# christhetree/mod_extraction

Measured on AMD Instinct MI355X. Metric: 44.1 kHz audio-seconds/sec (train step), interwoven ph/fl/ch, higher is better.
Workload: dtype f32

## Files before the change

mod_extraction_amd/csrc/phaser.hip:

```cpp
#include "phaser_common.h"

#define PH_BLOCK 256
#define PH_WPB 4

__global__ __launch_bounds__(64 * PH_WPB) void phaser_kernel(const float *__restrict__ x, long long x_stride,
                                                    const float *__restrict__ rate,
                                                    const float *__restrict__ depth,
                                                    const float *__restrict__ centre,
                                                    const float *__restrict__ feedback,
                                                    const float *__restrict__ mix,
                                                    const int *__restrict__ lead_arr,
                                                    const int *__restrict__ rows, int n_items, int N,
                                                    double sr, float *__restrict__ y, long long y_stride,
                                                    float *__restrict__ dry_out)
{
    const int lane = threadIdx.x & 63;
    const int item = blockIdx.x * PH_WPB + (threadIdx.x >> 6);
    if (item >= n_items) return;
    const int b = rows ? rows[item] : item;
    const int lead = lead_arr ? lead_arr[b] : 0;
    const int total = lead + N;
    const float *xb = x + (size_t)b * x_stride;
    float *yb = y + (size_t)b * y_stride;
    float *db = dry_out ? dry_out + (size_t)b * y_stride : nullptr;

    const PsClip k = ps_clip(sr, rate[b], depth[b], centre[b], feedback[b], mix[b]);

    float phase = 0.0f;
    float z[7] = {0.f, 0.f, 0.f, 0.f, 0.f, 0.f, 0.f};

    for (int n0 = 0; n0 < total; n0 += PH_BLOCK) {
        float xr[PH_BLOCK / 64], yr[PH_BLOCK / 64];
#pragma unroll
        for (int j = 0; j < PH_BLOCK / 64; ++j) {
            const int n = n0 + j * 64 + lane;
            xr[j] = n < total ? xb[n] : 0.0f;
            yr[j] = 0.0f;
        }
        float my_phase = 0.0f;
        for (int u = 0; u < PH_BLOCK / 4; ++u) {
            if (lane == u) my_phase = phase;
            phase = ps_step(phase, k.inc);
        }
        float pre_unused;
        const float Greg = ps_cutoff(k, ps_osc(my_phase), pre_unused);
        const int cnt = min(PH_BLOCK, total - n0);
#pragma unroll
        for (int j = 0; j < PH_BLOCK / 64; ++j) {
            const int lim = min(64, cnt - j * 64);
            for (int li = 0; li < lim; ++li) {
                const float in = __int_as_float(__builtin_amdgcn_readlane(__float_as_int(xr[j]), li));
                const float G = __int_as_float(__builtin_amdgcn_readlane(__float_as_int(Greg), (j * 64 + li) >> 2));
                const float out = ps_sample(G, k.fb, in, z);
                float m = __fadd_rn(__fmul_rn(out, k.wet_g), __fmul_rn(in, k.dry_g));
                m = m < -1.0f ? -1.0f : (m > 1.0f ? 1.0f : m);
                yr[j] = lane == li ? m : yr[j];
            }
        }
#pragma unroll
        for (int j = 0; j < PH_BLOCK / 64; ++j) {
            const int n = n0 + j * 64 + lane;
            if (n >= lead && n < total) {
                yb[n - lead] = yr[j];
                if (db) db[n - lead] = xr[j];
            }
        }
    }
}


__device__ float ps_phase_after(int g, float inc)
{
    const float two_pi = PS_TWO_PI;
    float p = 0.0f;
    int rem = g;
    while (rem > 0) {
        const float p1 = ps_step(p, inc);
        p = p1;
        if (--rem == 0) break;
        const float p2 = ps_step(p1, inc);
        p = p2;
        if (--rem == 0) break;
        const float p3 = ps_step(p2, inc);
        p = p3;
        if (--rem == 0) break;
        const float d1 = __fsub_rn(p2, p1), d2 = __fsub_rn(p3, p2);
        const int e1 = (__float_as_int(p1) >> 23) & 0xff, e2 = (__float_as_int(p2) >> 23) & 0xff, e3 = (__float_as_int(p3) >> 23) & 0xff;
        if (d1 == d2 && d2 > 0.0f && e1 == e2 && e2 == e3 && e3 > 0 && e3 < 0xfe) {
            const double edge = (double)__int_as_float((e3 + 1) << 23);
            const double lim = edge < (double)two_pi ? edge : (double)two_pi;
            long long j = (long long)floor((lim - (double)p3) / (double)d2) - 1;
            if (j > rem) j = rem;
            if (j > 0) {
                p = (float)((double)p3 + (double)j * (double)d2);
                rem -= (int)j;
            }
        }
    }
    return p;
}

template <bool STASH>
__global__ __launch_bounds__(PS_P) void phaser_scan_kernel(const float *__restrict__ x, long long x_stride,
                                                           const float *__restrict__ rate,
                                                           const float *__restrict__ depth,
                                                           const float *__restrict__ centre,
                                                           const float *__restrict__ feedback,
                                                           const float *__restrict__ mix,
                                                           const int *__restrict__ lead_arr,
                                                           const int *__restrict__ rows, int n_items, int N, double sr,
                                                           float *__restrict__ y, long long y_stride,
                                                           float *__restrict__ dry_out, float *__restrict__ gws,
                                                           long long gws_stride, int probe,
                                                           const float *__restrict__ mod, long long mod_stride, int n_mod,
                                                           float *__restrict__ stash, long long stash_stride, int sg,
                                                           int x_width)
{
    extern __shared__ __attribute__((aligned(16))) float ps_lds[];
    float *mv = ps_lds, *zs = ps_lds + PS_P * PS_MV;
    const int p = threadIdx.x, lane = p & 63;
    const int item = blockIdx.x;
    const int b = rows ? rows[item] : item;
    const int lead = lead_arr ? lead_arr[b] : 0;
    const int total = lead + N;
    const float *xb = x + (size_t)b * x_stride;
    float *yb = y + (size_t)b * y_stride;
    float *db = dry_out ? dry_out + (size_t)b * y_stride : nullptr;
    float *gw = gws + (size_t)item * gws_stride;
    PsStash<float> st = {nullptr, sg};
    const float *mb = nullptr;
    if constexpr (STASH) {
        if (total > x_width || ((total + 3) >> 2) > sg) return;
        st.row = stash + (size_t)b * stash_stride;
        gw = st.G();
        if (mod) mb = mod + (size_t)b * mod_stride;
    }
    const bool ext = STASH && mb != nullptr;

    const PsClip k = ps_clip(sr, ext ? 0.0f : rate[b], depth[b], centre[b], feedback[b], mix[b]);

    const int n_groups = (total + 3) >> 2;
    const int gpc = (n_groups + PS_P - 1) / PS_P;
    const int g0 = p * gpc, g1 = min(g0 + gpc, n_groups);

    const bool use_ws = STASH || (gws != nullptr && (long long)n_groups <= gws_stride);

    float S[8][7];
#pragma unroll
    for (int r = 0; r < 8; ++r)
#pragma unroll
        for (int c = 0; c < 7; ++c) S[r][c] = r == c ? 1.0f : 0.0f;
    float phase = ext ? 0.0f : ps_phase_after(min(g0, n_groups), k.inc);
    for (int g = g0; g < g1; ++g) {
        float xv[4];
#pragma unroll
        for (int j = 0; j < 4; ++j) {
            const int n = 4 * g + j;
            xv[j] = probe ? 0.25f : (n < total ? xb[n] : 0.0f);
        }
        float pre;
        const float osc = ext ? __fsub_rn(1.0f, __fmul_rn(2.0f, g < n_mod ? mb[g] : 0.5f)) : ps_osc(phase);
        const float G = ps_cutoff(k, osc, pre);
        if constexpr (STASH) {
            st.pre()[g] = pre;
            st.osc()[g] = osc;
        }
        phase = ps_step(phase, k.inc);
        if (use_ws) gw[g] = G;
#pragma unroll
        for (int j = 0; j < 4; ++j) {
#pragma unroll
            for (int r = 0; r < 8; ++r) (void)ps_sample(G, k.fb, r == 7 ? xv[j] : 0.0f, S[r]);
        }
    }
    {
        float *m = mv + p * PS_MV;
#pragma unroll
        for (int c = 0; c < 7; ++c)
#pragma unroll
            for (int r = 0; r < 7; ++r) m[c * 7 + r] = S[c][r];
#pragma unroll
        for (int r = 0; r < 7; ++r) m[49 + r] = S[7][r];
        if constexpr (STASH) m[PS_MV - 1] = 0.0f;
    }
    __syncthreads();

    if (p < 64) {
        const int r = lane < 7 ? lane : 0;
        float z[7], mine = 0.0f;
#pragma unroll
        for (int c = 0; c < 7; ++c) z[c] = 0.0f;
        for (int q = 0; q < PS_P; ++q) {
            if (lane < 7) zs[q * 8 + lane] = mine;
            const float *m = mv + q * PS_MV;
            float acc = m[49 + r];
#pragma unroll
            for (int c = 0; c < 7; ++c) acc = __builtin_fmaf(m[c * 7 + r], z[c], acc);
            mine = acc;
#pragma unroll
            for (int c = 0; c < 7; ++c) z[c] = __int_as_float(__builtin_amdgcn_readlane(__float_as_int(acc), c));
        }
    }
    __syncthreads();
    if constexpr (STASH) {
        for (int i = p; i < PS_P * PS_MV; i += PS_P) st.maps()[i] = mv[i];
        for (int g = n_groups + p; g < sg; g += PS_P) {
            st.G()[g] = 0.0f;
            st.pre()[g] = 0.0f;
            st.osc()[g] = 0.0f;
            st.pass()[g] = 0;
        }
        const float4 zero4 = make_float4(0.0f, 0.0f, 0.0f, 0.0f);
        const int spc = (gpc + PS_SUB - 1) / PS_SUB;
        for (int sub = (max(g1 - g0, 0) + PS_SUB - 1) / PS_SUB; sub < spc; ++sub) {
            float4 *ck = st.ckpt(p, gpc, sub);
            ck[0] = zero4;
            ck[1] = zero4;
        }
        float4 *ck_all = st.ckpt(0, gpc, 0);
        const long long ck_used = 2ll * PS_P * spc, ck_row = 2ll * PS_P * ps_ckpts_per_chunk(sg);
        for (long long i = ck_used + p; i < ck_row; i += PS_P) ck_all[i] = zero4;
    }

    {
        float z[7];
#pragma unroll
        for (int c = 0; c < 7; ++c) z[c] = zs[p * 8 + c];
        float phase_c = use_ws ? 0.0f : ps_phase_after(min(g0, n_groups), k.inc);
        for (int g = g0; g < g1; ++g) {
            float G;
            if (use_ws) G = gw[g];
            else {
                float pre_unused;
                G = ps_cutoff(k, ps_osc(phase_c), pre_unused);
                phase_c = ps_step(phase_c, k.inc);
            }
            float xv[4];
#pragma unroll
            for (int j = 0; j < 4; ++j) {
                const int n = 4 * g + j;
                xv[j] = probe ? 0.25f : (n < total ? xb[n] : 0.0f);
            }
            int passed = 0;
            if constexpr (STASH) {
                if (((g - g0) & (PS_SUB - 1)) == 0) {
                    float4 *ck = st.ckpt(p, gpc, (g - g0) / PS_SUB);
                    ck[0] = make_float4(z[0], z[1], z[2], z[3]);
                    ck[1] = make_float4(z[4], z[5], z[6], 0.0f);
                }
            }
#pragma unroll
            for (int j = 0; j < 4; ++j) {
                const int n = 4 * g + j;
                const float in = xv[j];
                const float out = ps_sample(G, k.fb, in, z);
                float m = __fadd_rn(__fmul_rn(out, k.wet_g), __fmul_rn(in, k.dry_g));
                if constexpr (STASH) passed |= (m >= -1.0f && m <= 1.0f) ? 1 << j : 0;
                m = m < -1.0f ? -1.0f : (m > 1.0f ? 1.0f : m);
                if (n >= lead && n < total && (!probe || g + 1 == g1)) {
                    yb[n - lead] = m;
                    if (db) db[n - lead] = in;
                }
            }
            if constexpr (STASH) st.pass()[g] = passed;
        }
    }
}

static int phaser_fwd_launch(const float *x, int64_t x_stride, const float *rate, const float *depth,
                            const float *centre, const float *feedback, const float *mix, const int32_t *lead,
                            const int32_t *rows, int64_t n_rows, int64_t B, int64_t N, double sr, int32_t exact_order,
                            float *y, int64_t y_stride, float *dry_out, float *workspace, int64_t workspace_stride,
                            void *stream, int probe)
{
    if (!x || !rate || !depth || !centre || !feedback || !mix || !y || B <= 0 || N <= 0 || sr <= 0.0) return MX_ERR_ARG;
    if (workspace && workspace_stride <= 0) return MX_ERR_ARG;
    if (N >= (1ll << 30)) return MX_ERR_UNSUPPORTED;
    const int64_t items = rows ? n_rows : B;
    if (items <= 0) return MX_OK;
    if (exact_order) {
        const dim3 grid((unsigned)((items + PH_WPB - 1) / PH_WPB)), block(64 * PH_WPB);
        hipLaunchKernelGGL(phaser_kernel, grid, block, 0, (hipStream_t)stream, x, (long long)x_stride, rate, depth, centre,
                           feedback, mix, lead, rows, (int)items, (int)N, sr, y, (long long)y_stride, dry_out);
    } else {
        const size_t lds = PS_LDS_FLOATS * sizeof(float);
        static MxLdsLatch latch = {};
        if (mx_set_dyn_lds(latch, (const void *)phaser_scan_kernel<false>, lds) != MX_OK) return MX_ERR_LAUNCH;
        hipLaunchKernelGGL(phaser_scan_kernel<false>, dim3((unsigned)items), dim3(PS_P), lds, (hipStream_t)stream, x, (long long)x_stride,
                           rate, depth, centre, feedback, mix, lead, rows, (int)items, (int)N, sr, y, (long long)y_stride,
                           dry_out, workspace, (long long)workspace_stride, probe, (const float *)nullptr, 0ll, 0,
                           (float *)nullptr, 0ll, 0, 0);
    }
    return mx_launch_status();
}

MX_EXPORT int mx_phaser_fwd(const float *x, int64_t x_stride, const float *rate, const float *depth,
                            const float *centre, const float *feedback, const float *mix, const int32_t *lead,
                            const int32_t *rows, int64_t n_rows, int64_t B, int64_t N, double sr, int32_t exact_order,
                            float *y, int64_t y_stride, float *dry_out, float *workspace, int64_t workspace_stride,
                            void *stream)
{
    return phaser_fwd_launch(x, x_stride, rate, depth, centre, feedback, mix, lead, rows, n_rows, B, N, sr, exact_order, y, y_stride, dry_out, workspace, workspace_stride, stream, 0);
}

MX_EXPORT int mx_phaser_fwd_stash(const float *x, int64_t x_stride, int64_t x_width, const float *mod, int64_t n_mod,
                                  const float *rate, const float *depth, const float *centre, const float *feedback,
                                  const float *mix, const int32_t *lead, const int32_t *rows, int64_t n_rows, int64_t B,
                                  int64_t N, double sr, float *y, int64_t y_stride, float *dry_out, float *stash,
                                  int64_t stash_groups, int64_t stash_stride, void *stream)
{
    if (!x || !(mod || rate) || !depth || !centre || !feedback || !mix || !y || !stash || B <= 0 || N <= 0 || sr <= 0.0)
        return MX_ERR_ARG;
    if (x_width < N || x_stride < x_width || y_stride < N || (mod && n_mod < (x_width + 3) / 4)) return MX_ERR_ARG;
    if (x_width >= (1ll << 30)) return MX_ERR_UNSUPPORTED;
    if (stash_groups < (x_width + 3) / 4 || (stash_groups & 3) || stash_stride < ps_stash_floats(stash_groups)) return MX_ERR_ARG;
    if ((stash_stride & 3) || ((uintptr_t)stash & 15)) return MX_ERR_ARG;
    const int64_t items = rows ? n_rows : B;
    if (items <= 0) return MX_OK;
    const size_t lds = PS_LDS_FLOATS * sizeof(float);
    static MxLdsLatch latch = {};
    if (mx_set_dyn_lds(latch, (const void *)phaser_scan_kernel<true>, lds) != MX_OK) return MX_ERR_LAUNCH;
    hipLaunchKernelGGL(phaser_scan_kernel<true>, dim3((unsigned)items), dim3(PS_P), lds, (hipStream_t)stream, x, (long long)x_stride,
                       rate, depth, centre, feedback, mix, lead, rows, (int)items, (int)N, sr, y, (long long)y_stride, dry_out,
                       (float *)nullptr, 0ll, 0, mod, (long long)n_mod, (int)n_mod, stash, (long long)stash_stride,
                       (int)stash_groups, (int)x_width);
    return mx_launch_status();
}

MX_EXPORT int mx_phaser_fwd_probe(const float *x, int64_t x_stride, const float *rate, const float *depth,
                            const float *centre, const float *feedback, const float *mix, const int32_t *lead,
                            const int32_t *rows, int64_t n_rows, int64_t B, int64_t N, double sr, int32_t exact_order,
                            float *y, int64_t y_stride, float *dry_out, float *workspace, int64_t workspace_stride,
                            void *stream)
{
    return phaser_fwd_launch(x, x_stride, rate, depth, centre, feedback, mix, lead, rows, n_rows, B, N, sr, exact_order, y, y_stride, dry_out, workspace, workspace_stride, stream, 1);
}

__global__ __launch_bounds__(PS_P) void phaser_cascade_probe_kernel(int steps, float G, float fb, float *__restrict__ out)
{
    float s[8][6], last[8];
#pragma unroll
    for (int r = 0; r < 8; ++r) {
        last[r] = 0.0f;
#pragma unroll
        for (int k = 0; k < 6; ++k) s[r][k] = (r == k) ? 1.0f : 0.001f * (float)(threadIdx.x & 7);
    }
    float in = 0.25f + 1e-3f * (float)(threadIdx.x & 15);
    for (int t = 0; t < steps; ++t) {
#pragma unroll
        for (int r = 0; r < 8; ++r) {
            float o = __fsub_rn(r == 7 ? in : 0.0f, last[r]);
#pragma unroll
            for (int k = 0; k < 6; ++k) (void)ps_stage(G, s[r][k], o);
            last[r] = __fmul_rn(o, fb);
        }
        in = -in;
    }
    float acc = 0.0f;
#pragma unroll
    for (int r = 0; r < 8; ++r) acc += last[r] + s[r][5];
    if (acc == 123.456f) out[threadIdx.x] = acc;
    if (threadIdx.x == 0) out[0] = acc;
}

MX_EXPORT int mx_phaser_cascade_probe(int64_t steps, float *out, void *stream)
{
    if (!out || steps <= 0 || steps >= (1ll << 30)) return MX_ERR_ARG;
    hipLaunchKernelGGL(phaser_cascade_probe_kernel, dim3(1), dim3(PS_P), 0, (hipStream_t)stream, (int)steps, 0.37f, 0.45f, out);
    return mx_launch_status();
}
```

mod_extraction_amd/csrc/phaser_common.h:

```cpp
#pragma once
#include "common.h"

#define PS_WAVES 8
#define PS_P (64 * PS_WAVES)
#define PS_MV 57
#define PS_LDS_FLOATS (PS_P * PS_MV + (PS_P + 1) * 8)
#define PS_SUB 2

__host__ __device__ inline long long ps_ckpts_per_chunk(long long n_groups)
{
    const long long gpc = (n_groups + PS_P - 1) / PS_P;
    return (gpc + PS_SUB - 1) / PS_SUB;
}
__host__ __device__ inline long long ps_stash_floats(long long sg)
{
    return 4 * sg + (long long)PS_P * PS_MV + (long long)PS_P * 8 * ps_ckpts_per_chunk(sg);
}

__device__ __forceinline__ int *ps_as_int(float *p) { return reinterpret_cast<int *>(p); }
__device__ __forceinline__ const int *ps_as_int(const float *p) { return reinterpret_cast<const int *>(p); }
__device__ __forceinline__ float4 *ps_as_float4(float *p) { return reinterpret_cast<float4 *>(p); }
__device__ __forceinline__ const float4 *ps_as_float4(const float *p) { return reinterpret_cast<const float4 *>(p); }
template <typename F>
struct PsStash {
    F *row;
    int sg;
    __device__ __forceinline__ F *G() const { return row; }
    __device__ __forceinline__ F *pre() const { return row + sg; }
    __device__ __forceinline__ F *osc() const { return row + 2 * (size_t)sg; }
    __device__ __forceinline__ auto pass() const { return ps_as_int(row) + 3 * (size_t)sg; }
    __device__ __forceinline__ F *maps() const { return row + 4 * (size_t)sg; }
    __device__ __forceinline__ auto ckpt(int p, int gpc, int sub) const
    {
        return ps_as_float4(maps() + PS_P * PS_MV) + 2 * ((size_t)p * ((gpc + PS_SUB - 1) / PS_SUB) + sub);
    }
};

constexpr float PS_TWO_PI = 6.283185307179586476925286766559f;
constexpr double PS_PI = 3.14159265358979323846;

struct PsClip {
    double sr;
    float log_min, span, inc, norm_centre, osc_vol, fb, wet_g, dry_g;
};
__device__ __forceinline__ PsClip ps_clip(double sr, float rate, float depth, float centre, float feedback, float mix)
{
    PsClip k;
    const float fmax_hz = (float)fmin(20000.0, 0.49 * sr);
    k.sr = sr;
    k.log_min = (float)log10(20.0);
    k.span = __fsub_rn((float)log10((double)fmax_hz), k.log_min);
    k.inc = __fmul_rn(__fdiv_rn(PS_TWO_PI, (float)(sr / 4.0)), rate);
    k.norm_centre = __fdiv_rn(__fsub_rn((float)log10((double)centre), k.log_min), k.span);
    k.osc_vol = __fmul_rn(depth, 0.5f);
    k.fb = feedback;
    k.wet_g = mix;
    k.dry_g = __fsub_rn(1.0f, mix);
    return k;
}

__device__ __forceinline__ float ps_step(float p, float inc)
{
    p = __fadd_rn(p, inc);
    while (p >= PS_TWO_PI) p = __fsub_rn(p, PS_TWO_PI);
    return p;
}
__device__ __forceinline__ float ps_osc(float phase) { return (float)sin((double)__fsub_rn(phase, (float)PS_PI)); }
__device__ __forceinline__ float ps_cutoff(const PsClip &k, float osc, float &pre)
{
    pre = __fadd_rn(__fmul_rn(osc, k.osc_vol), k.norm_centre);
    const float lfo = pre < 0.0f ? 0.0f : (pre > 1.0f ? 1.0f : pre);
    const float fc = (float)pow(10.0, (double)__fadd_rn(__fmul_rn(lfo, k.span), k.log_min));
    const float g = (float)tan(PS_PI * (double)fc / k.sr);
    return __fdiv_rn(g, __fadd_rn(1.0f, g));
}

__device__ __forceinline__ float ps_stage(float G, float &s, float &out)
{
    const float d = __fsub_rn(out, s);
    const float v = __fmul_rn(G, d);
    const float yk = __fadd_rn(v, s);
    s = __fadd_rn(v, yk);
    out = __fsub_rn(__fmul_rn(2.0f, yk), out);
    return d;
}
__device__ __forceinline__ float ps_sample(float G, float fb, float in, float (&z)[7], float *d = nullptr)
{
    float out = __fsub_rn(in, z[6]);
#pragma unroll
    for (int k = 0; k < 6; ++k) {
        const float dk = ps_stage(G, z[k], out);
        if (d) d[k] = dk;
    }
    z[6] = __fmul_rn(out, fb);
    return out;
}
```

Baseline: 7651.

## Precompute phaser cutoff table in a separate parallel kernel before scan

Adds a phaser_cutoff_kernel that fills the per-group cutoff coefficient table across a 2D grid, with each thread handling a short run of groups from a recomputed phase. The non-stash scan kernel then reads G from this table (prefetching the next value) instead of evaluating the double-precision sin/pow/tan chain inline. This moves the expensive transcendental work off the serial scan into a wide parallel pass. The cost is an extra launch and a global write/read of the table. In probe mode a fixed constant G stands in for the table.

New measurement: 7649 (median of 2 runs). No clear change (-0.0%).

```diff
diff --git a/mod_extraction_amd/csrc/phaser.hip b/mod_extraction_amd/csrc/phaser.hip
--- a/mod_extraction_amd/csrc/phaser.hip
+++ b/mod_extraction_amd/csrc/phaser.hip
@@ -42,8 +42,7 @@
             if (lane == u) my_phase = phase;
             phase = ps_step(phase, k.inc);
         }
-        float pre_unused;
-        const float Greg = ps_cutoff(k, ps_osc(my_phase), pre_unused);
+        const float Greg = ps_cutoff_at(k, my_phase);
         const int cnt = min(PH_BLOCK, total - n0);
 #pragma unroll
         for (int j = 0; j < PH_BLOCK / 64; ++j) {
@@ -100,6 +99,37 @@
     return p;
 }
 
+#define PC_BLOCK 256
+#define PC_RUN 8
+#define PS_PROBE_G 0.37f
+__global__ __launch_bounds__(PC_BLOCK) void phaser_cutoff_kernel(const float *__restrict__ rate,
+                                                                 const float *__restrict__ depth,
+                                                                 const float *__restrict__ centre,
+                                                                 const float *__restrict__ feedback,
+                                                                 const float *__restrict__ mix,
+                                                                 const int *__restrict__ lead_arr,
+                                                                 const int *__restrict__ rows, int N, double sr,
+                                                                 float *__restrict__ gws, long long gws_stride)
+{
+    const int item = blockIdx.x;
+    const int b = rows ? rows[item] : item;
+    const int lead = lead_arr ? lead_arr[b] : 0;
+    const int total = lead + N;
+    const int n_groups = (total + 3) >> 2;
+    if ((long long)n_groups > gws_stride) return;
+    float *gw = gws + (size_t)item * gws_stride;
+    const PsClip k = ps_clip(sr, rate[b], depth[b], centre[b], feedback[b], mix[b]);
+    const long long span = (long long)gridDim.y * (PC_BLOCK * PC_RUN);
+    for (long long first = ((long long)blockIdx.y * PC_BLOCK + threadIdx.x) * PC_RUN; first < n_groups; first += span) {
+        const int g0 = (int)first, g1 = min(g0 + PC_RUN, n_groups);
+        float phase = ps_phase_after(g0, k.inc);
+        for (int g = g0; g < g1; ++g) {
+            gw[g] = ps_cutoff_at(k, phase);
+            phase = ps_step(phase, k.inc);
+        }
+    }
+}
+
 template <bool STASH>
 __global__ __launch_bounds__(PS_P) void phaser_scan_kernel(const float *__restrict__ x, long long x_stride,
                                                            const float *__restrict__ rate,
@@ -144,13 +174,15 @@
     const int g0 = p * gpc, g1 = min(g0 + gpc, n_groups);
 
     const bool use_ws = STASH || (gws != nullptr && (long long)n_groups <= gws_stride);
+    const bool table = !STASH && use_ws;
 
     float S[8][7];
 #pragma unroll
     for (int r = 0; r < 8; ++r)
 #pragma unroll
         for (int c = 0; c < 7; ++c) S[r][c] = r == c ? 1.0f : 0.0f;
-    float phase = ext ? 0.0f : ps_phase_after(min(g0, n_groups), k.inc);
+    float phase = (ext || table) ? 0.0f : ps_phase_after(min(g0, n_groups), k.inc);
+    float G_next = (table && !probe && g0 < g1) ? gw[g0] : PS_PROBE_G;
     for (int g = g0; g < g1; ++g) {
         float xv[4];
 #pragma unroll
@@ -158,15 +190,21 @@
             const int n = 4 * g + j;
             xv[j] = probe ? 0.25f : (n < total ? xb[n] : 0.0f);
         }
-        float pre;
-        const float osc = ext ? __fsub_rn(1.0f, __fmul_rn(2.0f, g < n_mod ? mb[g] : 0.5f)) : ps_osc(phase);
-        const float G = ps_cutoff(k, osc, pre);
-        if constexpr (STASH) {
-            st.pre()[g] = pre;
-            st.osc()[g] = osc;
-        }
-        phase = ps_step(phase, k.inc);
-        if (use_ws) gw[g] = G;
+        float G;
+        if (table) {
+            G = G_next;
+            if (!probe && g + 1 < g1) G_next = gw[g + 1];
+        } else {
+            float pre;
+            const float osc = ext ? __fsub_rn(1.0f, __fmul_rn(2.0f, g < n_mod ? mb[g] : 0.5f)) : ps_osc(phase);
+            G = ps_cutoff(k, osc, pre);
+            if constexpr (STASH) {
+                st.pre()[g] = pre;
+                st.osc()[g] = osc;
+                gw[g] = G;
+            }
+            phase = ps_step(phase, k.inc);
+        }
 #pragma unroll
         for (int j = 0; j < 4; ++j) {
 #pragma unroll
@@ -229,10 +267,9 @@
         float phase_c = use_ws ? 0.0f : ps_phase_after(min(g0, n_groups), k.inc);
         for (int g = g0; g < g1; ++g) {
             float G;
-            if (use_ws) G = gw[g];
+            if (use_ws) G = (table && probe) ? PS_PROBE_G : gw[g];
             else {
-                float pre_unused;
-                G = ps_cutoff(k, ps_osc(phase_c), pre_unused);
+                G = ps_cutoff_at(k, phase_c);
                 phase_c = ps_step(phase_c, k.inc);
             }
             float xv[4];
@@ -286,6 +323,12 @@
         const size_t lds = PS_LDS_FLOATS * sizeof(float);
         static MxLdsLatch latch = {};
         if (mx_set_dyn_lds(latch, (const void *)phaser_scan_kernel<false>, lds) != MX_OK) return MX_ERR_LAUNCH;
+        if (workspace && !probe) {
+            const int64_t per_block = PC_BLOCK * PC_RUN, blocks = (workspace_stride - 1) / per_block + 1;
+            const dim3 grid((unsigned)items, (unsigned)(blocks < 65535 ? blocks : 65535));
+            hipLaunchKernelGGL(phaser_cutoff_kernel, grid, dim3(PC_BLOCK), 0, (hipStream_t)stream, rate, depth, centre, feedback,
+                               mix, lead, rows, (int)N, sr, workspace, (long long)workspace_stride);
+        }
         hipLaunchKernelGGL(phaser_scan_kernel<false>, dim3((unsigned)items), dim3(PS_P), lds, (hipStream_t)stream, x, (long long)x_stride,
                            rate, depth, centre, feedback, mix, lead, rows, (int)items, (int)N, sr, y, (long long)y_stride,
                            dry_out, workspace, (long long)workspace_stride, probe, (const float *)nullptr, 0ll, 0,
diff --git a/mod_extraction_amd/csrc/phaser_common.h b/mod_extraction_amd/csrc/phaser_common.h
--- a/mod_extraction_amd/csrc/phaser_common.h
+++ b/mod_extraction_amd/csrc/phaser_common.h
@@ -74,6 +74,11 @@
     const float g = (float)tan(PS_PI * (double)fc / k.sr);
     return __fdiv_rn(g, __fadd_rn(1.0f, g));
 }
+__device__ __forceinline__ float ps_cutoff_at(const PsClip &k, float phase)
+{
+    float pre_unused;
+    return ps_cutoff(k, ps_osc(phase), pre_unused);
+}
 
 __device__ __forceinline__ float ps_stage(float G, float &s, float &out)
 {
```
